# myshell-ai/OpenVoice

Measured on NVIDIA H100. Metric: audio_seconds_per_second, higher is better.
Workload: dtype f32 (3xFP16 split-precision tensor-core convs with fp32 accumulation, fp32 FFMA elsewhere)

## Files before the change

include/ovc.h:

```cpp
#ifndef OVC_B200_H
#define OVC_B200_H

#include <stddef.h>
#include <stdint.h>

#ifdef __cplusplus
extern "C" {
#endif

#define OVC_ABI_VERSION 11

#if defined(__GNUC__)
#define OVC_API __attribute__((visibility("default")))
#else
#define OVC_API
#endif

enum {
  OVC_OK = 0,
  OVC_ERR_INVALID = -1,
  OVC_ERR_CUDA = -2,
  OVC_ERR_STATE = -3,
  OVC_ERR_MISSING = -4,
  OVC_ERR_NOMEM = -5
};

typedef struct ovc_ctx ovc_ctx;

typedef struct ovc_hparams {
  int32_t spec_channels;
  int32_t inter_channels;
  int32_t hidden_channels;
  int32_t gin_channels;
// ... 91 lines not shown
                                 const ovc_item_params* items);

OVC_API int ovc_tts_encode_state(ovc_ctx* ctx, float* stats, int32_t* cum, float* g, void* stream);

OVC_API int ovc_tts_encode_state_rows(ovc_ctx* ctx, const int64_t* dst_row, int N, int Tp, float* stats, int32_t* cum,
                                      float* g, int64_t* y_lengths, void* stream);
OVC_API int ovc_tts_state_rows(ovc_ctx* ctx, const float* stats, const int32_t* cum, const float* g, const int64_t* y_lengths,
                               int B, int T, const int64_t* dst_row, int N, int Tp, float* d_stats, int32_t* d_cum,
                               float* d_g, int64_t* d_y_lengths, void* stream);

OVC_API int ovc_tts_decode_windows(ovc_ctx* ctx, const float* stats, const int32_t* cum, const float* g,
                                   const int64_t* y_lengths, int N, int T, const int64_t* row, const int64_t* frame0,
                                   const int64_t* len, int W, int Wmax, const uint64_t* seed, const int64_t* stream,
                                   const float* noise_scale, float* o, float* z_p, void* cuda_stream);

OVC_API int ovc_set_precision(ovc_ctx* ctx, int mode);

#define OVC_OPT_TTS_SIMPLE 2
#define OVC_OPT_GRAPH 3
#define OVC_OPT_PDL 5
#define OVC_OPT_BRANCHES 7
#define OVC_OPT_PAIR 8
#define OVC_OPT_PAIR_OCC 9
OVC_API int ovc_set_option(ovc_ctx* ctx, int key, int value);

OVC_API int ovc_last_launch_count(const ovc_ctx* ctx);

OVC_API int ovc_graph_replays(const ovc_ctx* ctx);

OVC_API int ovc_profile_enable(ovc_ctx* ctx, int enable);
OVC_API int ovc_profile_read(ovc_ctx* ctx, double* ms, int64_t* launches, double* flops, double* bytes);
OVC_API int ovc_profile_detail(ovc_ctx* ctx, int max, char* names, double* ms, double* flops, double* bytes,
                               int* family);

OVC_API int ovc_debug_enable(ovc_ctx* ctx, int enable);
OVC_API int ovc_debug_fetch(ovc_ctx* ctx, const char* name, float* host_out, size_t max_floats,
                    int64_t* shape4 );

#ifdef __cplusplus
}
#endif
#endif
```

openvoice_b200/_native.py:

```python
from __future__ import annotations

import ctypes as C
import os
from typing import Dict, Iterable, Optional, Tuple

_HERE = os.path.dirname(os.path.abspath(__file__))
LIB_PATH = os.path.join(_HERE, "libovc_b200.so")

ABI_VERSION = 11
EXPORTS = (
    "ovc_abi_version", "ovc_last_error", "ovc_create", "ovc_destroy", "ovc_load_tensor",
    "ovc_finalize_weights", "ovc_workspace_floats", "ovc_voice_conversion", "ovc_last_launch_count",
    "ovc_profile_enable", "ovc_profile_read", "ovc_profile_detail", "ovc_debug_enable", "ovc_debug_fetch",
    "ovc_spectrogram", "ovc_convert_waveform", "ovc_set_precision", "ovc_reference_encoder",
    "ovc_tts_info", "ovc_tts_encode", "ovc_tts_decode", "ovc_set_option", "ovc_graph_replays",
    "ovc_reference_encoder_ragged", "ovc_resample", "ovc_resample_span", "ovc_voice_conversion_items",
    "ovc_convert_waveform_items", "ovc_tts_encode_items", "ovc_tts_decode_items", "ovc_philox_normals",
    "ovc_tts_encode_state", "ovc_tts_decode_windows", "ovc_spectrogram_ring", "ovc_splice",
    "ovc_tts_encode_state_rows", "ovc_tts_state_rows",
)

STREAM_OPEN = 2 ** 63 - 1
SPLICE_PCM16 = 1


class OvcHParams(C.Structure):
    _fields_ = [
        ("spec_channels", C.c_int32), ("inter_channels", C.c_int32), ("hidden_channels", C.c_int32),
        ("gin_channels", C.c_int32), ("resblock", C.c_int32), ("n_resblock_kernels", C.c_int32),
        ("resblock_kernel_sizes", C.c_int32 * 4), ("resblock_dilations", (C.c_int32 * 3) * 4),
        ("n_upsamples", C.c_int32), ("upsample_rates", C.c_int32 * 4),
        ("upsample_kernel_sizes", C.c_int32 * 4), ("upsample_initial_channel", C.c_int32),
# ... 208 lines not shown
        used, ignored = [], []
        for k, v in sd.items():
            a = v.detach().cpu().float().contiguous().numpy() if hasattr(v, "detach") else np.ascontiguousarray(v, dtype=np.float32)
            if a.ndim == 0 or a.ndim > 4:
                ignored.append(k)
                continue
            shape = (C.c_int64 * a.ndim)(*a.shape)
            rc = self.lib.ovc_load_tensor(self.handle, k.encode(), a.ctypes.data_as(C.c_void_p), shape, a.ndim)
            _check(self.lib, rc, f"ovc_load_tensor({k})")
            (ignored if rc == 1 else used).append(k)
        self.finalized = False
        return used, ignored

    def finalize(self):
        _check(self.lib, self.lib.ovc_finalize_weights(self.handle), "ovc_finalize_weights")
        self.finalized = True

    def set_precision(self, mode: str):
        m = PRECISIONS[mode]
        _check(self.lib, self.lib.ovc_set_precision(self.handle, m), "ovc_set_precision")
        self.precision = mode

    def set_option(self, key: str, value: int):
        k = {"tts_simple": 2, "graph": 3, "pdl": 5, "branches": 7, "pair": 8, "pair_occ": 9}[key]
        _check(self.lib, self.lib.ovc_set_option(self.handle, k, int(value)), "ovc_set_option")

    def voice_conversion(self, spec, lengths, g_src, g_tgt, noise=None, tau: float = 0.3, seed: int = 0,
                         ragged: bool = False, latents: bool = True, stream=None, items: Optional[dict] = None, out=None):
        import torch
        assert spec.is_cuda and spec.dtype == torch.float32 and spec.is_contiguous()
        assert lengths.is_cuda and lengths.dtype == torch.int64 and lengths.is_contiguous()
        B, S, T = spec.shape
        gs = g_src.reshape(B, -1).contiguous().float()
        gt = g_tgt.reshape(B, -1).contiguous().float()
        if noise is not None:
            noise = noise.contiguous().float()
            assert tuple(noise.shape) == (B, self.hp.inter_channels, T)
        hop = self.hp.hop_length
        if out is not None:
            assert out.is_cuda and out.dtype == torch.float32 and out.is_contiguous() and out.numel() == B * hop * T
            o = out.view(B, 1, hop * T)
        else:
            o = torch.empty(B, 1, hop * T, device=spec.device, dtype=torch.float32)
        lat = None
        if latents:
            lat = tuple(torch.empty(B, self.hp.inter_channels, T, device=spec.device, dtype=torch.float32)
                        for _ in range(3))
# ... 332 lines not shown
```

openvoice_b200/csrc/ovc_lib.cu:

```cuda
#include <cuda_runtime.h>

#include <algorithm>
#include <cmath>
#include <cstdarg>
#include <cstdio>
#include <cstdlib>
#include <cstring>
#include <map>
#include <string>
#include <vector>

#include "../../include/ovc.h"
#include "ovc_convpack.h"
#include "ovc_small.cuh"
#include "ovc_tcconv.cuh"
#include "ovc_tts.cuh"
#include "ovc_refenc.cuh"
#include "ovc_resample.cuh"
#include "ovc_splice.h"
#include "ovc_variants.h"

namespace ovc {

static thread_local std::string g_err;
// ... 126 lines not shown
  bool finalized = false;

  float* d_w = nullptr;
  size_t w_floats = 0;
  std::vector<float> h_w;

  ConvLayer enc_pre, enc_pre16, enc_proj;
  WNLayers enc_wn;
  ConvLayer flow_pre[4], flow_post[4];
  WNLayers flow_wn[4];
  ConvLayer dec_pre, dec_ups[4];
  ConvLayer rb_c1[12][3], rb_c2[12][3];
  TcLayer tc_c1[12][3], tc_c2[12][3], tc_ups[4], tc_pre;
  float* d_tcw = nullptr;
  std::vector<float> h_tcw;
  int precision = 0;
  bool tts_simple = false;
  bool use_graph = true;
  int use_pdl = 2;
  bool use_branches = true;
  int par_frames = 512;
  bool use_pair = true;
  bool use_pair_occ = true;
  bool pair_occ2_ok[TCN_N_OCC2] = {};
  cudaStream_t br_stream[2] = {nullptr, nullptr};
  cudaEvent_t br_ev[4] = {nullptr, nullptr, nullptr, nullptr};
  size_t post_w_off = 0;
  size_t cond_w_off = 0, cond_b_off = 0;
  int* d_cond_wrow = nullptr;
  int* d_cond_sel = nullptr;
  int cond_rows_out = 0;
  int cond_off_enc = 0, cond_off_fsrc = 0, cond_off_ftgt = 0, cond_off_dec = 0;
  int cond_off_enc_tc = 0, cond_off_fsrc_tc = 0, cond_off_ftgt_tc = 0;

  float2* d_tw = nullptr;
  float* d_win = nullptr;

  bool has_refenc = false;
  size_t re_conv_w[6] = {0}, re_conv_b[6] = {0}, re_wih = 0, re_whh = 0, re_bih = 0, re_bhh = 0, re_pw = 0, re_pb = 0,
         re_lng = 0, re_lnb = 0;
  int re_gru_in = 0;
  float* d_re = nullptr;
  size_t re_floats = 0;

  std::map<std::pair<int64_t, int64_t>, double*> rs_banks;
  bool rs_smem_opt_in = false;
// ... 365 lines not shown
        {"ref_enc.gru.weight_ih_l0", {384, c->re_gru_in}, &c->re_wih}, {"ref_enc.gru.weight_hh_l0", {384, 128}, &c->re_whh},
        {"ref_enc.gru.bias_ih_l0", {384}, &c->re_bih},                 {"ref_enc.gru.bias_hh_l0", {384}, &c->re_bhh},
        {"ref_enc.proj.weight", {G, 128}, &c->re_pw},                  {"ref_enc.proj.bias", {G}, &c->re_pb},
        {"ref_enc.layernorm.weight", {S}, &c->re_lng},                 {"ref_enc.layernorm.bias", {S}, &c->re_lnb}};
    for (const auto& e : re) {
      const HostTensor* t;
      TRY(tensor(c, e.key, e.shape, &t));
      *e.off = append(c->h_w, t->data);
    }
    c->has_refenc = true;
  }
  c->tts = TtsLayers();
  if (find(c, "enc_p.emb.weight")) TRY(pack_tts(c));
  ON_DEVICE(c);
  if (c->d_w) { cudaFree(c->d_w); c->d_w = nullptr; }
  c->w_floats = c->h_w.size();
  CK(cudaMalloc(&c->d_w, c->w_floats * sizeof(float)));
  CK(cudaMemcpy(c->d_w, c->h_w.data(), c->w_floats * sizeof(float), cudaMemcpyHostToDevice));
  if (c->d_tcw) { cudaFree(c->d_tcw); c->d_tcw = nullptr; }
  CK(cudaMalloc(&c->d_tcw, c->h_tcw.size() * sizeof(float)));
  CK(cudaMemcpy(c->d_tcw, c->h_tcw.data(), c->h_tcw.size() * sizeof(float), cudaMemcpyHostToDevice));
  c->h_tcw.clear();
  c->h_tcw.shrink_to_fit();
  CK(cudaFuncSetAttribute(tcconv_kernel<128, false>, cudaFuncAttributeMaxDynamicSharedMemorySize, (int)TcnCfg<128, false>::SMEM_BYTES));
  CK(cudaFuncSetAttribute(tcconv_kernel<64, false>, cudaFuncAttributeMaxDynamicSharedMemorySize, (int)TcnCfg<64, false>::SMEM_BYTES));
  CK(cudaFuncSetAttribute(tcconv_kernel<32, false>, cudaFuncAttributeMaxDynamicSharedMemorySize, (int)TcnCfg<32, false>::SMEM_BYTES));
  CK(cudaFuncSetAttribute(tcconv_kernel<128, true>, cudaFuncAttributeMaxDynamicSharedMemorySize, (int)TcnCfg<128, true>::SMEM_BYTES));
  CK(cudaFuncSetAttribute(tcconv_kernel<64, true>, cudaFuncAttributeMaxDynamicSharedMemorySize, (int)TcnCfg<64, true>::SMEM_BYTES));
  CK(cudaFuncSetAttribute(tcconv_kernel<32, true>, cudaFuncAttributeMaxDynamicSharedMemorySize, (int)TcnCfg<32, true>::SMEM_BYTES));
  for (int i = 0; i < TCN_N_OCC2; ++i) {
    const TcPairKernel k = tc_pair_kernel(kTcPairOcc2[i].C, kTcPairOcc2[i].o);
    CK(cudaFuncSetAttribute(k.fn, cudaFuncAttributeMaxDynamicSharedMemorySize, (int)k.smem));
    int blocks = 0;
    CK(cudaOccupancyMaxActiveBlocksPerMultiprocessor(&blocks, k.fn, TCN_THREADS, k.smem));
    c->pair_occ2_ok[i] = blocks >= 2;
    if (blocks < 2)
      fprintf(stderr, "ovc: the C = %d conv-pair kernel with %d operand buffer(s) fits %d CTA(s) per SM, not 2; its pairs run "
              "one CTA per SM\n", kTcPairOcc2[i].C, kTcPairOcc2[i].o.nabuf, blocks);
  }
  if (c->d_cond_wrow) cudaFree(c->d_cond_wrow);
  if (c->d_cond_sel) cudaFree(c->d_cond_sel);
  CK(cudaMalloc(&c->d_cond_wrow, wrow.size() * sizeof(int)));
  CK(cudaMalloc(&c->d_cond_sel, sel.size() * sizeof(int)));
  CK(cudaMemcpy(c->d_cond_wrow, wrow.data(), wrow.size() * sizeof(int), cudaMemcpyHostToDevice));
  CK(cudaMemcpy(c->d_cond_sel, sel.data(), sel.size() * sizeof(int), cudaMemcpyHostToDevice));
  if (!c->d_tw) {
    std::vector<float2> tw(STFT_N);
    std::vector<float> win(STFT_N);
    const double PI = 3.14159265358979323846;
    for (int m = 0; m < STFT_N; ++m) {
      tw[m] = make_float2((float)std::cos(2.0 * PI * m / STFT_N), (float)(-std::sin(2.0 * PI * m / STFT_N)));
      win[m] = (float)(0.5 - 0.5 * std::cos(2.0 * PI * m / STFT_N));
    }
    CK(cudaMalloc(&c->d_tw, STFT_N * sizeof(float2)));
    CK(cudaMalloc(&c->d_win, STFT_N * sizeof(float)));
    CK(cudaMemcpy(c->d_tw, tw.data(), STFT_N * sizeof(float2), cudaMemcpyHostToDevice));
    CK(cudaMemcpy(c->d_win, win.data(), STFT_N * sizeof(float), cudaMemcpyHostToDevice));
// ... 175 lines not shown
static int launch_tc(Run& r, const TcLayer& T, const float* x, float* y, const float* res, int t_len, int mul, float slope,
                     float scale, int accumulate, int family, const TcExtra& ex = TcExtra()) {
  TcConvArgs a{};
  const int y_ld = ex.y_ld ? ex.y_ld : T.Ntot;
  a.x = x; a.x_bs = (long long)T.Cin * r.P * mul;
  a.w = reinterpret_cast<const uint16_t*>(r.c->d_tcw + T.w_off);
  a.bias = ex.bias ? ex.bias : r.c->d_tcw + T.b_off; a.bias_bs = ex.bias_bs;
  a.y = y; a.y_bs = (long long)y_ld * r.P * mul; a.y_ld = y_ld;
  a.r = res;
  a.s = ex.s; a.s_bs = a.y_bs;
  a.epi = ex.epi; a.split = ex.split; a.first = ex.first;
  a.lens = ex.use_lens_frames ? r.lens : r.glens; a.tmax = r.Tmax; a.mul = mul;
  a.lens_x = ex.lens_x; a.has_lens_x = ex.has_lens_x ? 1 : 0;
  a.Cin = T.Cin; a.Ntot = T.Ntot; a.K = T.K; a.DIL = T.DIL;
  a.slope = slope; a.scale = scale; a.accumulate = accumulate;
  a.passes = r.c->precision == 2 ? 1 : 3;
  if (T.TN == 0) return fail(OVC_ERR_INVALID, "conv %d -> %d (k %d, dilation %d) does not fit the tensor-core kernels", T.Cin, T.Ntot, T.K, T.DIL);
  if (!(slope >= 0.f && slope <= 1.f)) return fail(OVC_ERR_INVALID, "leaky_relu slope %g outside [0, 1]", (double)slope);
  TRY(prof_begin(r));
  const TcGrid g = tc_grid(t_len, r.B, T.Ntot, T.TN, r.c->sm_count, ex.grid_div);
  const int n_tt = g.n_tt, total = g.total;
  dim3 pg((unsigned)g.grid_x, g.ncol, 1);
  const bool pdl = r.c->use_pdl == 1 || (r.c->use_pdl == 2 && ex.epi != 0);
  if (T.TN == 128) CK(launch_ex(tcconv_kernel<128, false>, pg, TCN_THREADS, TcnCfg<128, false>::SMEM_BYTES, r.st, pdl, a, n_tt, total));
  else if (T.TN == 64) CK(launch_ex(tcconv_kernel<64, false>, pg, TCN_THREADS, TcnCfg<64, false>::SMEM_BYTES, r.st, pdl, a, n_tt, total));
  else CK(launch_ex(tcconv_kernel<32, false>, pg, TCN_THREADS, TcnCfg<32, false>::SMEM_BYTES, r.st, pdl, a, n_tt, total));
  CK(cudaGetLastError());
  r.c->launches++;
  const double units = (double)r.B * t_len;
  const int eff_k = family == 2 ? 2 : T.K;
  TRY(prof_end(r, T.TN == 128 ? V_TC128 : T.TN == 64 ? V_TC64 : V_TC32, family == 1 ? 1 : 0, 2.0 * T.Cin * T.Ntot * eff_k * units,
               4.0 * (T.Cin + T.Ntot * (1 + (res ? 1 : 0) + (accumulate ? 1 : 0))) * units, (T.Cin << 16) | (T.K << 8) | T.DIL));
  return OVC_OK;
}

static int launch_pair(Run& r, const TcLayer& T1, const TcLayer& T2, const float* x, float* y, int t_len, int mul, float slope,
                       float scale, int accumulate) {
  TcConvArgs a{};
  const int C = T1.TN;
  a.x = x; a.x_bs = (long long)C * r.P * mul;
  a.w = reinterpret_cast<const uint16_t*>(r.c->d_tcw + T1.w_off);
  a.w2 = reinterpret_cast<const uint16_t*>(r.c->d_tcw + T2.w_off);
  a.bias = r.c->d_tcw + T1.b_off; a.bias2 = r.c->d_tcw + T2.b_off;
  a.y = y; a.y_bs = a.x_bs; a.y_ld = C;
  a.lens = r.glens; a.tmax = r.Tmax; a.mul = mul;
  a.Cin = C; a.Ntot = C; a.K = T1.K; a.DIL = T1.DIL;
  a.slope = slope; a.scale = scale; a.accumulate = accumulate;
  a.passes = r.c->precision == 2 ? 1 : 3;
  TcPairOcc o = r.c->use_pair_occ ? tc_pair_occ(T1, T2) : TcPairOcc();
  for (int i = 0; i < TCN_N_OCC2; ++i)
    if (o.occ == 2 && kTcPairOcc2[i].C == C && kTcPairOcc2[i].o.nabuf == o.nabuf && !r.c->pair_occ2_ok[i]) o = TcPairOcc();
  const TcPairKernel k = tc_pair_kernel(C, o);
  if (!k.fn) return fail(OVC_ERR_INVALID, "no conv-pair kernel for C = %d at %d CTA(s) per SM, %d operand buffer(s)", C, o.occ, o.nabuf);
  const TcGrid g = tc_pair_grid(t_len, r.B, T1.K, r.c->sm_count, o.occ);
  const int n_tt = g.n_tt, total = g.total;
  TRY(prof_begin(r));
  dim3 pg((unsigned)g.grid_x, 1, 1);
  CK(launch_ex(k.fn, pg, TCN_THREADS, k.smem, r.st, false, a, n_tt, total));
  CK(cudaGetLastError());
  r.c->launches++;
  const double units = (double)r.B * t_len;
  TRY(prof_end(r, C == 128 ? V_TCPAIR128 : C == 64 ? V_TCPAIR64 : V_TCPAIR32, 1, 2.0 * 2.0 * C * C * T1.K * units, 4.0 * C * (2 + (accumulate ? 1 : 0)) * units,
               (C << 16) | (T1.K << 8) | T1.DIL));
  return OVC_OK;
}

static int launch_transpose(Run& r, const float* src, float* dst, int rows, int cols) {
  dim3 grid((cols + 31) / 32, (rows + 31) / 32, r.B);
  TRY(prof_begin(r));
  transpose_kernel<<<grid, 256, 0, r.st>>>(src, dst, rows, cols, (long long)rows * cols);
  CK(cudaGetLastError());
  r.c->launches++;
  TRY(prof_end(r, V_TRANSPOSE, 0, 0.0, 8.0 * rows * cols * r.B));
  return OVC_OK;
}

static int run_wn(Run& r, const WNLayers& wn, float* x, float* skip, float* acts, const float* cond, int cond_bs) {
  const int P = r.P, T = r.Tmax;
  const long long bs = 192LL * P;
  const int n = (int)wn.in.size();
  for (int i = 0; i < n; ++i) {
// ... 138 lines not shown
  }
  const cudaError_t ie = cudaGraphInstantiate(&e->exec, graph, 0);
  cudaGraphDestroy(graph);
  if (ie != cudaSuccess) {
    cudaGetLastError();
    e->exec = nullptr;
    e->seen = -1000000;
    return body(st);
  }
  e->launches = c->launches;
  CK(cudaGraphLaunch(e->exec, st));
  c->graph_replays++;
  return OVC_OK;
}

static int set_call_params(ovc_ctx* c, uint64_t seed, float tau, const ItemParams& items, cudaStream_t st) {
  if (!c->d_callp) CK(cudaMalloc(&c->d_callp, sizeof(CallParams)));
  set_call_params_kernel<<<1, 1, 0, st>>>(c->d_callp, seed, tau, items);
  CK(cudaGetLastError());
  return OVC_OK;
}
static uintptr_t option_bits(const ovc_ctx* c) {
  return (uintptr_t)c->precision | ((uintptr_t)c->use_pdl << 15) | ((uintptr_t)c->use_branches << 14) | ((uintptr_t)c->use_pair << 17) |
         ((uintptr_t)c->use_pair_occ << 18);
}

static int ensure_ws(ovc_ctx* c, const WsLayout& W, int B, int Tmax, cudaStream_t st) {
  if (W.total <= c->ws_floats) return OVC_OK;
  CK(cudaStreamSynchronize(st));
  drop_graphs(c);
  if (c->d_ws) CK(cudaFree(c->d_ws));
  c->d_ws = nullptr;
  c->ws_floats = 0;
  cudaError_t e = cudaMalloc(&c->d_ws, W.total * sizeof(float));
  if (e != cudaSuccess) {
    cudaGetLastError();
    return fail(OVC_ERR_NOMEM, "workspace of %.2f GB for B=%d Tmax=%d does not fit: %s", W.total * 4e-9, B, Tmax,
                cudaGetErrorString(e));
  }
  c->ws_floats = W.total;
  return OVC_OK;
}

static int copy_latent_out(Run& r, const WsLayout& W, float* ws, float* dst) {
  if (!dst) return OVC_OK;
  dim3 grid((r.Tmax + 255) / 256, 192, r.B);
  copy_latent_kernel<<<grid, 256, 0, r.st>>>(ws + W.z, W.P, dst, r.Tmax, 192, r.lens);
// ... 727 lines not shown
  CK(cudaGetLastError());
  return OVC_OK;
}

int ovc_set_precision(ovc_ctx* c, int mode) {
  if (!c) return fail(OVC_ERR_INVALID, "null context");
  if (mode < 0 || mode > 2) return fail(OVC_ERR_INVALID, "precision mode must be 0 (fp32 FFMA), 1 (3xFP16 tensor cores) or 2 (single-pass fp16)");
  c->precision = mode;
  return OVC_OK;
}

int ovc_set_option(ovc_ctx* c, int key, int value) {
  if (!c) return fail(OVC_ERR_INVALID, "null context");
  switch (key) {
    case OVC_OPT_TTS_SIMPLE: c->tts_simple = value != 0; return OVC_OK;
    case OVC_OPT_GRAPH: c->use_graph = value != 0; return OVC_OK;
    case OVC_OPT_PDL:
      if (value < 0 || value > 2) return fail(OVC_ERR_INVALID, "pdl must be 0, 1 or 2");
      c->use_pdl = value;
      return OVC_OK;
    case OVC_OPT_BRANCHES: c->use_branches = value != 0; return OVC_OK;
    case OVC_OPT_PAIR: c->use_pair = value != 0; return OVC_OK;
    case OVC_OPT_PAIR_OCC: c->use_pair_occ = value != 0; return OVC_OK;
    default: return fail(OVC_ERR_INVALID, "unknown option %d", key);
  }
}

int ovc_last_launch_count(const ovc_ctx* c) { return c ? c->launches : 0; }

int ovc_graph_replays(const ovc_ctx* c) { return c ? c->graph_replays : 0; }

int ovc_profile_enable(ovc_ctx* c, int enable) {
  if (!c) return fail(OVC_ERR_INVALID, "null context");
  c->prof = enable != 0;
  c->ev_used = 0;
  c->ev_flops.clear();
  c->ev_bytes.clear();
  c->ev_variant.clear();
  c->ev_family.clear();
  c->ev_tag.clear();
  return OVC_OK;
}

int ovc_profile_read(ovc_ctx* c, double* ms, int64_t* launches, double* flops, double* bytes) {
  if (!c) return fail(OVC_ERR_INVALID, "null context");
  double tms = 0, tf = 0, tb = 0;
// ... 68 lines not shown
```

openvoice_b200/csrc/ovc_tcconv.cuh:

```cuda
#pragma once
#include "ovc_conv.cuh"
#include "ovc_tc.cuh"
#include "ovc_tcpack.h"

namespace ovc {

struct TcConvArgs {
  const float* x; long long x_bs;
  const uint16_t* w;
  const float* bias; long long bias_bs;
  float* y; long long y_bs; int y_ld;
  const float* r;
  float* s; long long s_bs;
  int epi;
  int split; int first;
  const long long* lens; int tmax; int mul;
  const long long* lens_x; int has_lens_x;
  int Cin; int Ntot; int K; int DIL;
  float slope; float scale; int accumulate;
  int passes;
  const uint16_t* w2; const float* bias2;
};

__device__ __forceinline__ void pdl_launch_dependents() { asm volatile("griddepcontrol.launch_dependents;" ::: "memory"); }
__device__ __forceinline__ void pdl_wait() { asm volatile("griddepcontrol.wait;" ::: "memory"); }

__device__ __forceinline__ void mbar_arrive(uint64_t* bar) {
  asm volatile("mbarrier.arrive.shared::cta.b64 _, [%0];" ::"r"(smem_u32(bar)) : "memory");
}
__device__ __forceinline__ void named_bar_sync(int id, int threads) {
  asm volatile("bar.sync %0, %1;" ::"r"(id), "r"(threads) : "memory");
}

template <int TN>
__device__ __forceinline__ void tc_epilogue(const TcConvArgs& a, const float (&d)[TN], int b, int t0, int n0, int lim, int row_a) {
  const int csub = (threadIdx.x & 3) * 2;
  float* yb = a.y + (size_t)b * a.y_bs;
  const float* rb = a.r ? a.r + (size_t)b * a.y_bs : nullptr;
  float* sb = a.s ? a.s + (size_t)b * a.s_bs : nullptr;
  const float* bias = a.bias + (size_t)b * a.bias_bs;
  const bool two = a.passes == 3;
  const int ta = t0 + row_a, tb = ta + 8;
  const bool oka = ta < lim, okb = tb < lim;
#pragma unroll
  for (int c0 = 0; c0 < TN; c0 += 32) {
    float v[16];
#pragma unroll
    for (int i = 0; i < 16; ++i) v[i] = two ? fmaf(d[TN / 2 + c0 / 2 + i], tc::kLoInv, d[c0 / 2 + i]) : d[c0 / 2 + i];
#pragma unroll
    for (int g = 0; g < 4; ++g) {
      const float2 bq = __ldg(reinterpret_cast<const float2*>(bias + n0 + c0 + 8 * g + csub));
      v[4 * g] += bq.x; v[4 * g + 1] += bq.y; v[4 * g + 2] += bq.x; v[4 * g + 3] += bq.y;
    }
    if (a.epi == 0) {
      float* ypa = yb + (size_t)ta * a.y_ld + n0 + c0 + csub;
      float* ypb = yb + (size_t)tb * a.y_ld + n0 + c0 + csub;
      const float* rpa = rb ? rb + (size_t)ta * a.y_ld + n0 + c0 + csub : nullptr;
      const float* rpb = rb ? rb + (size_t)tb * a.y_ld + n0 + c0 + csub : nullptr;
#pragma unroll
      for (int g = 0; g < 4; ++g) {
        float2 oa = make_float2(v[4 * g], v[4 * g + 1]), ob = make_float2(v[4 * g + 2], v[4 * g + 3]);
        if (rb) {
          const float2 qa = oka ? *reinterpret_cast<const float2*>(rpa + 8 * g) : make_float2(0.f, 0.f);
          const float2 qb = okb ? *reinterpret_cast<const float2*>(rpb + 8 * g) : make_float2(0.f, 0.f);
          oa.x += qa.x; oa.y += qa.y; ob.x += qb.x; ob.y += qb.y;
        }
        if (a.accumulate) {
          const float2 ya = oka ? *reinterpret_cast<const float2*>(ypa + 8 * g) : make_float2(0.f, 0.f);
          const float2 yc = okb ? *reinterpret_cast<const float2*>(ypb + 8 * g) : make_float2(0.f, 0.f);
          oa.x = ya.x + oa.x; oa.y = ya.y + oa.y;
          ob.x = yc.x + ob.x; ob.y = yc.y + ob.y;
// ... 14 lines not shown
        if (oka) *reinterpret_cast<float2*>(ypa + 8 * g) = oa;
        if (okb) *reinterpret_cast<float2*>(ypb + 8 * g) = ob;
      }
    } else {
      const int col = n0 + c0;
      const bool to_x = col < a.split;
      const bool add = to_x || !a.first;
      float* dst = (to_x ? yb + col : sb + (col - a.split)) + csub;
#pragma unroll
      for (int g = 0; g < 4; ++g) {
        float2 oa = make_float2(v[4 * g], v[4 * g + 1]), ob = make_float2(v[4 * g + 2], v[4 * g + 3]);
        if (add) {
          const float2 qa = oka ? *reinterpret_cast<const float2*>(dst + (size_t)ta * a.y_ld + 8 * g) : make_float2(0.f, 0.f);
          const float2 qb = okb ? *reinterpret_cast<const float2*>(dst + (size_t)tb * a.y_ld + 8 * g) : make_float2(0.f, 0.f);
          oa = make_float2(qa.x + oa.x, qa.y + oa.y);
          ob = make_float2(qb.x + ob.x, qb.y + ob.y);
        }
        if (oka) *reinterpret_cast<float2*>(dst + (size_t)ta * a.y_ld + 8 * g) = oa;
        if (okb) *reinterpret_cast<float2*>(dst + (size_t)tb * a.y_ld + 8 * g) = ob;
      }
    }
  }
}

template <int TN>
__device__ __forceinline__ void tc_mma_step(float (&d)[TN], uint64_t a_hi, uint64_t a_lo, uint64_t b, bool three, bool first) {
  float (&lo)[TN / 2] = *reinterpret_cast<float(*)[TN / 2]>(&d[TN / 2]);
  float (&hi)[TN / 2] = *reinterpret_cast<float(*)[TN / 2]>(&d[0]);
  tc::Wgmma<TN>::mma(hi, a_hi, b, first ? 0 : 1);
  if (three) {
    tc::Wgmma<TN>::mma(lo, a_hi, b + TN, first ? 0 : 1);
    tc::Wgmma<TN>::mma(lo, a_lo, b, 1);
  }
}

constexpr int TCN_THREADS = 384;
constexpr int TCN_NCT = 96;

template <int TN, bool PAIR, int OCC = 1, int NAB = 2>
struct TcnCfg {
  static_assert(!PAIR || TN == 32 || TN == 64 || TN == 128, "conv pairs: C = 32, 64 or 128");
  static_assert(OCC == 1 || (PAIR && TN <= 64), "two CTAs per SM: C = 32 / 64 pairs");
  static constexpr int KCH = 32, NKC = KCH / 8;
  static constexpr int ROWS = 194;
  static constexpr int ROWS2 = TCN_ROWS2;
  static constexpr int NABUF = NAB;
  static constexpr int RING = PAIR ? tc_pair_ring(TN, OCC, NAB) : tc_ring_slots(TN, PAIR);
  static constexpr int SLOT_BYTES = 2 * 2 * TN * 16;
  static constexpr int A_BUF_BYTES = 2 * NKC * ROWS * 16;
  static constexpr int A2_BYTES = PAIR ? 2 * (TN / 8) * ROWS2 * 16 : 0;
  static constexpr size_t SMEM_BYTES = 1024 + NABUF * A_BUF_BYTES + A2_BYTES + RING * SLOT_BYTES;
  static_assert(!PAIR || SMEM_BYTES == tc_pair_smem(TN, NABUF, RING), "tc_pair_smem");
  static_assert(SMEM_BYTES <= (OCC == 1 ? 232448 : TCN_SMEM_OCC2), "shared memory budget");
  static_assert((2 * NABUF + 2 * RING) * 8 <= 1024, "barrier area");
  static constexpr int PROD_REGS = OCC == 1 ? 56 : 32, MMA_REGS = OCC == 1 ? 224 : 104;
};

template <int TN, bool PAIR, int OCC = 1, int NAB = 2>
__global__ void __launch_bounds__(TCN_THREADS, OCC) tcconv_kernel(const TcConvArgs a, int n_tt, int total) {
  using Cfg = TcnCfg<TN, PAIR, OCC, NAB>;
  constexpr int ROWS = Cfg::ROWS, ROWS2 = Cfg::ROWS2, NABUF = Cfg::NABUF, RING = Cfg::RING, NKC = Cfg::NKC;
  extern __shared__ __align__(128) unsigned char smem_raw[];
  uint64_t* bars = reinterpret_cast<uint64_t*>(smem_raw);
  uint64_t *a_full = bars, *a_empty = bars + NABUF, *b_full = a_empty + NABUF, *b_empty = b_full + RING;
  unsigned char* abuf = smem_raw + 1024;
  unsigned char* a2buf = abuf + NABUF * Cfg::A_BUF_BYTES;
  unsigned char* bring = a2buf + Cfg::A2_BYTES;

  const int tid = threadIdx.x, lane = tid & 31;
  const int warp = __shfl_sync(0xffffffffu, tid >> 5, 0);
  const int H1 = (a.K - 1) / 2 * a.DIL;
  const int H2 = PAIR ? (a.K - 1) / 2 : 0;
  const int R = 128 - 2 * H2;
  const int rows8 = (128 + 2 * H1 + 7) & ~7;
  const int nq = a.Cin / Cfg::KCH;
  const int n_slots = (a.Cin / 16) * a.K;
  const int n_w = PAIR ? 2 * n_slots : n_slots;
  const bool resident = n_w <= RING;
  if (H1 > TCN_HMAX || (PAIR && 128 + 2 * H2 > ROWS2)) __trap();
  constexpr uint32_t BYTES = Cfg::SLOT_BYTES;

  if (tid == 0) {
    for (int i = 0; i < NABUF; ++i) { mbar_init(&a_full[i], TCN_NCT); mbar_init(&a_empty[i], 2); }
    for (int i = 0; i < RING; ++i) { mbar_init(&b_full[i], 1); mbar_init(&b_empty[i], 2); }
    fence_mbar_init();
  }
  if (PAIR) {
    for (int i = tid; i < Cfg::A2_BYTES / 16; i += TCN_THREADS) reinterpret_cast<uint4*>(a2buf)[i] = make_uint4(0u, 0u, 0u, 0u);
    asm volatile("fence.proxy.async.shared::cta;" ::: "memory");
  }
  __syncthreads();
  pdl_launch_dependents();
  if (warp != 0) pdl_wait();

#define TCN_FOR_TILES                                                                                   \
  for (int tile = blockIdx.x; tile < total; tile += gridDim.x) {                                        \
    const int b = tile / n_tt, t0 = (tile % n_tt) * R;                                                  \
    const int lim = (a.lens ? (int)min((long long)a.tmax, a.lens[b]) : a.tmax) * a.mul;                 \
    const int lim_x = a.has_lens_x ? (int)min((long long)a.tmax, a.lens_x[b]) * a.mul : lim;            \
    (void)lim_x;                                                                                        \
    if (t0 >= lim) continue;

  if (warp < 4) {
    tc::regs_dealloc<Cfg::PROD_REGS>();
    if (warp == 0) {
      if (lane == 0) {
        const unsigned char* wt = reinterpret_cast<const unsigned char*>(a.w) + (size_t)blockIdx.y * n_slots * BYTES;
        if (resident) {
          for (int it = 0; it < n_w; ++it) {
            const unsigned char* src = it < n_slots ? wt + (size_t)it * BYTES
                                                    : reinterpret_cast<const unsigned char*>(a.w2) + (size_t)(it - n_slots) * BYTES;
// ... 42 lines not shown
              if (i < items && t >= 0 && t < lim_x) {
                const float4* src = reinterpret_cast<const float4*>(xb + (size_t)t * a.Cin + q * Cfg::KCH + kc * 8);
                v0[u] = src[0];
                v1[u] = src[1];
              }
            }
#pragma unroll
            for (int u = 0; u < PB; ++u) {
              const int i = i0 + TCN_NCT * u;
              if (i >= items) break;
              const int row = i >> 2, kc = i & 3;
              uint4 hi, lo;
              tc::split_f16x8(v0[u], v1[u], a.slope, hi, lo);
              *reinterpret_cast<uint4*>(ah + (kc * ROWS + row) * 16) = hi;
              *reinterpret_cast<uint4*>(al + (kc * ROWS + row) * 16) = lo;
            }
          }
          asm volatile("fence.proxy.async.shared::cta;" ::: "memory");
          mbar_arrive(&a_full[buf]);
          if (++buf == NABUF) { buf = 0; ephase ^= 1; }
        }
      }
    }
  } else {
    tc::regs_alloc<Cfg::MMA_REGS>();
    const int wg = (warp >> 2) - 1;
    const bool leader = (tid & 127) == 0;
    const int row_a = 64 * wg + 16 * (warp & 3) + (lane >> 2);
    constexpr uint32_t LBO_A = ROWS * 16, LBO_A2 = ROWS2 * 16, LBO_B = 2 * TN * 16, SBO = 128;
    constexpr uint32_t A_LO16 = (NKC * ROWS * 16) >> 4, A2_LO16 = ((TN / 8) * ROWS2 * 16) >> 4, SLOT16 = BYTES >> 4;
    const uint64_t a_proto = tc::make_desc(0, LBO_A, SBO), b_proto = tc::make_desc(0, LBO_B, SBO);
    const uint64_t b_ring = b_proto + (tc::smem_addr(bring) >> 4);
    const bool three = a.passes == 3;
    float d[TN];
#pragma unroll
    for (int i = 0; i < TN; ++i) d[i] = 0.f;
    if (resident)
      for (int it = 0; it < n_w; ++it) mbar_wait(&b_full[it], 0u);
    int slot = 0, buf = 0;
    uint32_t bphase = 0, aphase = 0;
    TCN_FOR_TILES
      (void)lim_x;
      bool first = true;
      if (resident) slot = 0;
      for (int q = 0; q < nq; ++q) {
        mbar_wait(&a_full[buf], aphase);
        tc::fence_regs(d);
        tc::wgmma_fence();
        int prev = -1;
        for (int j = 0; j < 2; ++j) {
          uint64_t a_cur = a_proto + ((tc::smem_addr(abuf + buf * Cfg::A_BUF_BYTES) + 64 * wg * 16 + 2 * j * LBO_A) >> 4);
          for (int tap = 0; tap < a.K; ++tap) {
            if (!resident) mbar_wait(&b_full[slot], bphase);
            tc_mma_step<TN>(d, a_cur, a_cur + A_LO16, b_ring + (uint32_t)slot * SLOT16, three, first);
            tc::wgmma_commit();
            if (!resident) {
              tc::wgmma_wait<1>();
              if (leader && prev >= 0) mbar_arrive(&b_empty[prev]);
              prev = slot;
            }
            first = false;
            a_cur += a.DIL;
            if (++slot == RING) { slot = 0; bphase ^= 1; }
          }
        }
        tc::wgmma_wait<0>();
        tc::fence_regs(d);
        if (leader) {
          if (prev >= 0) mbar_arrive(&b_empty[prev]);
          mbar_arrive(&a_empty[buf]);
        }
        if (++buf == NABUF) { buf = 0; aphase ^= 1; }
      }
      if constexpr (!PAIR) {
        tc_epilogue<TN>(a, d, b, t0, blockIdx.y * TN, lim, row_a);
      } else {
        named_bar_sync(1, 256);
        unsigned char* a2h = a2buf;
        unsigned char* a2l = a2buf + (TN / 8) * ROWS2 * 16;
        const int ta = t0 - H2 + row_a, tb = ta + 8;
        const bool oka = ta >= 0 && ta < lim, okb = tb >= 0 && tb < lim;
        const int csub = (lane & 3) * 2;
#pragma unroll
        for (int g = 0; g < TN / 8; ++g) {
          const float2 bq = __ldg(reinterpret_cast<const float2*>(a.bias + 8 * g + csub));
          float x[4];
#pragma unroll
          for (int i = 0; i < 4; ++i) x[i] = (three ? fmaf(d[TN / 2 + 4 * g + i], tc::kLoInv, d[4 * g + i]) : d[4 * g + i]) + ((i & 1) ? bq.y : bq.x);
          x[0] = oka ? fmaxf(x[0], x[0] * a.slope) : 0.f;
          x[1] = oka ? fmaxf(x[1], x[1] * a.slope) : 0.f;
          x[2] = okb ? fmaxf(x[2], x[2] * a.slope) : 0.f;
          x[3] = okb ? fmaxf(x[3], x[3] * a.slope) : 0.f;
          const __half2 ha = __floats2half2_rn(x[0], x[1]), hb = __floats2half2_rn(x[2], x[3]);
          const float2 fa = __half22float2(ha), fb = __half22float2(hb);
          const __half2 la = __floats2half2_rn((x[0] - fa.x) * tc::kLoScale, (x[1] - fa.y) * tc::kLoScale);
          const __half2 lb = __floats2half2_rn((x[2] - fb.x) * tc::kLoScale, (x[3] - fb.y) * tc::kLoScale);
          const int oa = (g * ROWS2 + row_a) * 16 + (lane & 3) * 4, ob = oa + 8 * 16;
          *reinterpret_cast<__half2*>(a2h + oa) = ha;
          *reinterpret_cast<__half2*>(a2h + ob) = hb;
          *reinterpret_cast<__half2*>(a2l + oa) = la;
// ... 8 lines not shown
        int prev = -1;
        for (int kk = 0; kk < TN / 16; ++kk) {
          uint64_t a_cur = a2_proto + ((tc::smem_addr(a2buf) + 64 * wg * 16 + 2 * kk * LBO_A2) >> 4);
          for (int tap = 0; tap < a.K; ++tap) {
            if (resident) {
              tc_mma_step<TN>(d, a_cur, a_cur + A2_LO16, b_ring + (uint32_t)(n_slots + kk * a.K + tap) * SLOT16, three, first2);
            } else {
              mbar_wait(&b_full[slot], bphase);
              tc_mma_step<TN>(d, a_cur, a_cur + A2_LO16, b_ring + (uint32_t)slot * SLOT16, three, first2);
              tc::wgmma_commit();
              tc::wgmma_wait<1>();
              if (leader && prev >= 0) mbar_arrive(&b_empty[prev]);
              prev = slot;
              if (++slot == RING) { slot = 0; bphase ^= 1; }
            }
            first2 = false;
            a_cur += 1;
          }
        }
        tc::wgmma_commit();
        tc::wgmma_wait<0>();
        tc::fence_regs(d);
        if (leader && prev >= 0) mbar_arrive(&b_empty[prev]);
        TcConvArgs e = a;
        e.y_ld = TN; e.r = a.x; e.bias = a.bias2; e.bias_bs = 0; e.epi = 0;
        tc_epilogue<TN>(e, d, b, t0, 0, min(lim, t0 + R), row_a);
      }
    }
  }
#undef TCN_FOR_TILES
}

struct TcPairKernel {
  void (*fn)(TcConvArgs, int, int) = nullptr;
  size_t smem = 0;
};
inline TcPairKernel tc_pair_kernel(int C, TcPairOcc o) {
  if (o.occ == 1 && o.nabuf == 2) {
    if (C == 128) return {tcconv_kernel<128, true>, TcnCfg<128, true>::SMEM_BYTES};
    if (C == 64) return {tcconv_kernel<64, true>, TcnCfg<64, true>::SMEM_BYTES};
    if (C == 32) return {tcconv_kernel<32, true>, TcnCfg<32, true>::SMEM_BYTES};
  } else if (o.occ == 2) {
    if (C == 32 && o.nabuf == 2) return {tcconv_kernel<32, true, 2, 2>, TcnCfg<32, true, 2, 2>::SMEM_BYTES};
    if (C == 32 && o.nabuf == 1) return {tcconv_kernel<32, true, 2, 1>, TcnCfg<32, true, 2, 1>::SMEM_BYTES};
    if (C == 64 && o.nabuf == 1) return {tcconv_kernel<64, true, 2, 1>, TcnCfg<64, true, 2, 1>::SMEM_BYTES};
  }
  return {};
}
constexpr int TCN_N_OCC2 = 3;
constexpr struct { int C; TcPairOcc o; } kTcPairOcc2[TCN_N_OCC2] = {{32, {2, 2}}, {32, {2, 1}}, {64, {2, 1}}};

template <int C>
__global__ void __launch_bounds__(256) conv_post_cl_kernel(const float* __restrict__ x, long long x_bs,
                                                           const float* __restrict__ w, float* __restrict__ y,
                                                           long long y_bs, int y_len, const long long* lens, int tmax,
                                                           int mul) {
  constexpr int TB = 256, ROWS = TB + 6, LD = ROWS + 3;
  __shared__ float ws[7][C];
  __shared__ float xs[C][LD];
  for (int i = threadIdx.x; i < C * 7; i += blockDim.x) ws[i % 7][i / 7] = w[i];
  const int b = blockIdx.y;
  const int lim = (lens ? (int)min((long long)tmax, lens[b]) : tmax) * mul;
  const int t0 = blockIdx.x * TB;
  const float* xb = x + (size_t)b * x_bs;
  for (int idx = threadIdx.x; idx < ROWS * (C / 4); idx += blockDim.x) {
    const int row = idx / (C / 4), q = idx % (C / 4);
    const int tt = t0 - 3 + row;
    float4 v = make_float4(0.f, 0.f, 0.f, 0.f);
// ... 40 lines not shown
```

Baseline: 2312.

## Add warp-specialized staged epilogue for TN=128 tensor-core convs

Adds a fourth warpgroup of store warps to the TN=128 conv and conv-pair kernels. The MMA warps now write their finished accumulators to a shared-memory staging tile and signal an mbarrier, and the store warps run the bias, activation and residual epilogue while the MMA warps start the next tile. The aim is to overlap epilogue global stores with tensor-core work. In exchange, MMA registers drop from 224 to 184, producer registers shrink, more shared memory is used, and extra barrier syncs are added. It is enabled by default only when passes*K >= 15.

```diff
diff --git a/include/ovc.h b/include/ovc.h
--- a/include/ovc.h
+++ b/include/ovc.h
@@ -8,7 +8,7 @@
 extern "C" {
 #endif
 
-#define OVC_ABI_VERSION 11
+#define OVC_ABI_VERSION 12
 
 #if defined(__GNUC__)
 #define OVC_API __attribute__((visibility("default")))
@@ -146,6 +146,7 @@
 #define OVC_OPT_BRANCHES 7
 #define OVC_OPT_PAIR 8
 #define OVC_OPT_PAIR_OCC 9
+#define OVC_OPT_STAGED_EPI 10
 OVC_API int ovc_set_option(ovc_ctx* ctx, int key, int value);
 
 OVC_API int ovc_last_launch_count(const ovc_ctx* ctx);
diff --git a/openvoice_b200/_native.py b/openvoice_b200/_native.py
--- a/openvoice_b200/_native.py
+++ b/openvoice_b200/_native.py
@@ -7,7 +7,7 @@
 _HERE = os.path.dirname(os.path.abspath(__file__))
 LIB_PATH = os.path.join(_HERE, "libovc_b200.so")
 
-ABI_VERSION = 11
+ABI_VERSION = 12
 EXPORTS = (
     "ovc_abi_version", "ovc_last_error", "ovc_create", "ovc_destroy", "ovc_load_tensor",
     "ovc_finalize_weights", "ovc_workspace_floats", "ovc_voice_conversion", "ovc_last_launch_count",
@@ -262,7 +262,7 @@
         self.precision = mode
 
     def set_option(self, key: str, value: int):
-        k = {"tts_simple": 2, "graph": 3, "pdl": 5, "branches": 7, "pair": 8, "pair_occ": 9}[key]
+        k = {"tts_simple": 2, "graph": 3, "pdl": 5, "branches": 7, "pair": 8, "pair_occ": 9, "staged_epi": 10}[key]
         _check(self.lib, self.lib.ovc_set_option(self.handle, k, int(value)), "ovc_set_option")
 
     def voice_conversion(self, spec, lengths, g_src, g_tgt, noise=None, tau: float = 0.3, seed: int = 0,
diff --git a/openvoice_b200/csrc/ovc_lib.cu b/openvoice_b200/csrc/ovc_lib.cu
--- a/openvoice_b200/csrc/ovc_lib.cu
+++ b/openvoice_b200/csrc/ovc_lib.cu
@@ -172,6 +172,7 @@
   int par_frames = 512;
   bool use_pair = true;
   bool use_pair_occ = true;
+  bool use_staged_epi = true;
   bool pair_occ2_ok[TCN_N_OCC2] = {};
   cudaStream_t br_stream[2] = {nullptr, nullptr};
   cudaEvent_t br_ev[4] = {nullptr, nullptr, nullptr, nullptr};
@@ -583,17 +584,17 @@
   CK(cudaMemcpy(c->d_tcw, c->h_tcw.data(), c->h_tcw.size() * sizeof(float), cudaMemcpyHostToDevice));
   c->h_tcw.clear();
   c->h_tcw.shrink_to_fit();
-  CK(cudaFuncSetAttribute(tcconv_kernel<128, false>, cudaFuncAttributeMaxDynamicSharedMemorySize, (int)TcnCfg<128, false>::SMEM_BYTES));
-  CK(cudaFuncSetAttribute(tcconv_kernel<64, false>, cudaFuncAttributeMaxDynamicSharedMemorySize, (int)TcnCfg<64, false>::SMEM_BYTES));
-  CK(cudaFuncSetAttribute(tcconv_kernel<32, false>, cudaFuncAttributeMaxDynamicSharedMemorySize, (int)TcnCfg<32, false>::SMEM_BYTES));
-  CK(cudaFuncSetAttribute(tcconv_kernel<128, true>, cudaFuncAttributeMaxDynamicSharedMemorySize, (int)TcnCfg<128, true>::SMEM_BYTES));
-  CK(cudaFuncSetAttribute(tcconv_kernel<64, true>, cudaFuncAttributeMaxDynamicSharedMemorySize, (int)TcnCfg<64, true>::SMEM_BYTES));
-  CK(cudaFuncSetAttribute(tcconv_kernel<32, true>, cudaFuncAttributeMaxDynamicSharedMemorySize, (int)TcnCfg<32, true>::SMEM_BYTES));
+  for (int TN : {128, 64, 32})
+    for (bool staged : {false, true}) {
+      const TcKernel k = tc_conv_kernel(TN, staged), p = tc_pair_kernel(TN, TcPairOcc(), staged);
+      CK(cudaFuncSetAttribute(k.fn, cudaFuncAttributeMaxDynamicSharedMemorySize, (int)k.smem));
+      CK(cudaFuncSetAttribute(p.fn, cudaFuncAttributeMaxDynamicSharedMemorySize, (int)p.smem));
+    }
   for (int i = 0; i < TCN_N_OCC2; ++i) {
-    const TcPairKernel k = tc_pair_kernel(kTcPairOcc2[i].C, kTcPairOcc2[i].o);
+    const TcKernel k = tc_pair_kernel(kTcPairOcc2[i].C, kTcPairOcc2[i].o);
     CK(cudaFuncSetAttribute(k.fn, cudaFuncAttributeMaxDynamicSharedMemorySize, (int)k.smem));
     int blocks = 0;
-    CK(cudaOccupancyMaxActiveBlocksPerMultiprocessor(&blocks, k.fn, TCN_THREADS, k.smem));
+    CK(cudaOccupancyMaxActiveBlocksPerMultiprocessor(&blocks, k.fn, k.threads, k.smem));
     c->pair_occ2_ok[i] = blocks >= 2;
     if (blocks < 2)
       fprintf(stderr, "ovc: the C = %d conv-pair kernel with %d operand buffer(s) fits %d CTA(s) per SM, not 2; its pairs run "
@@ -815,9 +816,8 @@
   const int n_tt = g.n_tt, total = g.total;
   dim3 pg((unsigned)g.grid_x, g.ncol, 1);
   const bool pdl = r.c->use_pdl == 1 || (r.c->use_pdl == 2 && ex.epi != 0);
-  if (T.TN == 128) CK(launch_ex(tcconv_kernel<128, false>, pg, TCN_THREADS, TcnCfg<128, false>::SMEM_BYTES, r.st, pdl, a, n_tt, total));
-  else if (T.TN == 64) CK(launch_ex(tcconv_kernel<64, false>, pg, TCN_THREADS, TcnCfg<64, false>::SMEM_BYTES, r.st, pdl, a, n_tt, total));
-  else CK(launch_ex(tcconv_kernel<32, false>, pg, TCN_THREADS, TcnCfg<32, false>::SMEM_BYTES, r.st, pdl, a, n_tt, total));
+  const TcKernel k = tc_conv_kernel(T.TN, r.c->use_staged_epi && tc_stage_pays(T.K, a.passes));
+  CK(launch_ex(k.fn, pg, k.threads, k.smem, r.st, pdl, a, n_tt, total));
   CK(cudaGetLastError());
   r.c->launches++;
   const double units = (double)r.B * t_len;
@@ -843,13 +843,13 @@
   TcPairOcc o = r.c->use_pair_occ ? tc_pair_occ(T1, T2) : TcPairOcc();
   for (int i = 0; i < TCN_N_OCC2; ++i)
     if (o.occ == 2 && kTcPairOcc2[i].C == C && kTcPairOcc2[i].o.nabuf == o.nabuf && !r.c->pair_occ2_ok[i]) o = TcPairOcc();
-  const TcPairKernel k = tc_pair_kernel(C, o);
+  const TcKernel k = tc_pair_kernel(C, o, r.c->use_staged_epi && tc_stage_pays(T1.K, a.passes));
   if (!k.fn) return fail(OVC_ERR_INVALID, "no conv-pair kernel for C = %d at %d CTA(s) per SM, %d operand buffer(s)", C, o.occ, o.nabuf);
   const TcGrid g = tc_pair_grid(t_len, r.B, T1.K, r.c->sm_count, o.occ);
   const int n_tt = g.n_tt, total = g.total;
   TRY(prof_begin(r));
   dim3 pg((unsigned)g.grid_x, 1, 1);
-  CK(launch_ex(k.fn, pg, TCN_THREADS, k.smem, r.st, false, a, n_tt, total));
+  CK(launch_ex(k.fn, pg, k.threads, k.smem, r.st, false, a, n_tt, total));
   CK(cudaGetLastError());
   r.c->launches++;
   const double units = (double)r.B * t_len;
@@ -1034,7 +1034,7 @@
 }
 static uintptr_t option_bits(const ovc_ctx* c) {
   return (uintptr_t)c->precision | ((uintptr_t)c->use_pdl << 15) | ((uintptr_t)c->use_branches << 14) | ((uintptr_t)c->use_pair << 17) |
-         ((uintptr_t)c->use_pair_occ << 18);
+         ((uintptr_t)c->use_pair_occ << 18) | ((uintptr_t)c->use_staged_epi << 19);
 }
 
 static int ensure_ws(ovc_ctx* c, const WsLayout& W, int B, int Tmax, cudaStream_t st) {
@@ -1808,6 +1808,7 @@
     case OVC_OPT_BRANCHES: c->use_branches = value != 0; return OVC_OK;
     case OVC_OPT_PAIR: c->use_pair = value != 0; return OVC_OK;
     case OVC_OPT_PAIR_OCC: c->use_pair_occ = value != 0; return OVC_OK;
+    case OVC_OPT_STAGED_EPI: c->use_staged_epi = value != 0; return OVC_OK;
     default: return fail(OVC_ERR_INVALID, "unknown option %d", key);
   }
 }
diff --git a/openvoice_b200/csrc/ovc_tcconv.cuh b/openvoice_b200/csrc/ovc_tcconv.cuh
--- a/openvoice_b200/csrc/ovc_tcconv.cuh
+++ b/openvoice_b200/csrc/ovc_tcconv.cuh
@@ -31,22 +31,29 @@
 __device__ __forceinline__ void named_bar_sync(int id, int threads) {
   asm volatile("bar.sync %0, %1;" ::"r"(id), "r"(threads) : "memory");
 }
+__device__ __forceinline__ void named_bar_arrive(int id, int threads) {
+  asm volatile("bar.arrive %0, %1;" ::"r"(id), "r"(threads) : "memory");
+}
 
 template <int TN>
-__device__ __forceinline__ void tc_epilogue(const TcConvArgs& a, const float (&d)[TN], int b, int t0, int n0, int lim, int row_a) {
+__device__ __forceinline__ float tc_result(const float (&d)[TN], bool two, int j) {
+  return two ? fmaf(d[TN / 2 + j], tc::kLoInv, d[j]) : d[j];
+}
+
+template <int TN, class V>
+__device__ __forceinline__ void tc_epilogue_v(const TcConvArgs& a, V v_at, int b, int t0, int n0, int lim, int row_a) {
   const int csub = (threadIdx.x & 3) * 2;
   float* yb = a.y + (size_t)b * a.y_bs;
   const float* rb = a.r ? a.r + (size_t)b * a.y_bs : nullptr;
   float* sb = a.s ? a.s + (size_t)b * a.s_bs : nullptr;
   const float* bias = a.bias + (size_t)b * a.bias_bs;
-  const bool two = a.passes == 3;
   const int ta = t0 + row_a, tb = ta + 8;
   const bool oka = ta < lim, okb = tb < lim;
 #pragma unroll
   for (int c0 = 0; c0 < TN; c0 += 32) {
     float v[16];
 #pragma unroll
-    for (int i = 0; i < 16; ++i) v[i] = two ? fmaf(d[TN / 2 + c0 / 2 + i], tc::kLoInv, d[c0 / 2 + i]) : d[c0 / 2 + i];
+    for (int i = 0; i < 16; ++i) v[i] = v_at(c0 / 2 + i);
 #pragma unroll
     for (int g = 0; g < 4; ++g) {
       const float2 bq = __ldg(reinterpret_cast<const float2*>(bias + n0 + c0 + 8 * g + csub));
@@ -107,6 +114,16 @@
     }
   }
 }
+template <int TN>
+__device__ __forceinline__ void tc_epilogue(const TcConvArgs& a, const float (&d)[TN], int b, int t0, int n0, int lim, int row_a) {
+  const bool two = a.passes == 3;
+  tc_epilogue_v<TN>(a, [&](int j) { return tc_result<TN>(d, two, j); }, b, t0, n0, lim, row_a);
+}
+__device__ __forceinline__ TcConvArgs tc_pair_epilogue_args(const TcConvArgs& a, int TN) {
+  TcConvArgs e = a;
+  e.y_ld = TN; e.r = a.x; e.bias = a.bias2; e.bias_bs = 0; e.epi = 0;
+  return e;
+}
 
 template <int TN>
 __device__ __forceinline__ void tc_mma_step(float (&d)[TN], uint64_t a_hi, uint64_t a_lo, uint64_t b, bool three, bool first) {
@@ -122,10 +139,12 @@
 constexpr int TCN_THREADS = 384;
 constexpr int TCN_NCT = 96;
 
-template <int TN, bool PAIR, int OCC = 1, int NAB = 2>
+template <int TN, bool PAIR, int OCC = 1, int NAB = 2, bool STAGED = false>
 struct TcnCfg {
   static_assert(!PAIR || TN == 32 || TN == 64 || TN == 128, "conv pairs: C = 32, 64 or 128");
   static_assert(OCC == 1 || (PAIR && TN <= 64), "two CTAs per SM: C = 32 / 64 pairs");
+  static_assert(!STAGED || (TN == 128 && OCC == 1), "staged epilogue: TN = 128, one CTA per SM");
+  static constexpr int THREADS = STAGED ? TCN_THREADS + 128 : TCN_THREADS;
   static constexpr int KCH = 32, NKC = KCH / 8;
   static constexpr int ROWS = 194;
   static constexpr int ROWS2 = TCN_ROWS2;
@@ -134,23 +153,30 @@
   static constexpr int SLOT_BYTES = 2 * 2 * TN * 16;
   static constexpr int A_BUF_BYTES = 2 * NKC * ROWS * 16;
   static constexpr int A2_BYTES = PAIR ? 2 * (TN / 8) * ROWS2 * 16 : 0;
-  static constexpr size_t SMEM_BYTES = 1024 + NABUF * A_BUF_BYTES + A2_BYTES + RING * SLOT_BYTES;
+  static constexpr int STAGE_BYTES = STAGED ? (TN / 2) * 256 * 4 : 0;
+  static_assert(!STAGED || !PAIR || STAGE_BYTES <= A2_BYTES, "a pair's staging tile lies in its conv-2 operand");
+  static constexpr int SBUF_BYTES = STAGED && !PAIR ? STAGE_BYTES : 0;
+  static constexpr size_t SMEM_BYTES = 1024 + NABUF * A_BUF_BYTES + A2_BYTES + RING * SLOT_BYTES + SBUF_BYTES;
   static_assert(!PAIR || SMEM_BYTES == tc_pair_smem(TN, NABUF, RING), "tc_pair_smem");
   static_assert(SMEM_BYTES <= (OCC == 1 ? 232448 : TCN_SMEM_OCC2), "shared memory budget");
-  static_assert((2 * NABUF + 2 * RING) * 8 <= 1024, "barrier area");
-  static constexpr int PROD_REGS = OCC == 1 ? 56 : 32, MMA_REGS = OCC == 1 ? 224 : 104;
+  static_assert((2 * NABUF + 2 * RING + 2) * 8 <= 1024, "barrier area");
+  static constexpr int PROD_REGS = OCC == 1 && !STAGED ? 56 : 32, MMA_REGS = STAGED ? 184 : OCC == 1 ? 224 : 104;
+  static constexpr int STORE_REGS = 112;
+  static_assert(128 * PROD_REGS + 256 * MMA_REGS + (STAGED ? 128 * STORE_REGS : 0) <= 65536 / OCC, "register budget");
 };
 
-template <int TN, bool PAIR, int OCC = 1, int NAB = 2>
-__global__ void __launch_bounds__(TCN_THREADS, OCC) tcconv_kernel(const TcConvArgs a, int n_tt, int total) {
-  using Cfg = TcnCfg<TN, PAIR, OCC, NAB>;
+template <int TN, bool PAIR, int OCC = 1, int NAB = 2, bool STAGED = false>
+__global__ void __launch_bounds__(TcnCfg<TN, PAIR, OCC, NAB, STAGED>::THREADS, OCC) tcconv_kernel(const TcConvArgs a, int n_tt, int total) {
+  using Cfg = TcnCfg<TN, PAIR, OCC, NAB, STAGED>;
   constexpr int ROWS = Cfg::ROWS, ROWS2 = Cfg::ROWS2, NABUF = Cfg::NABUF, RING = Cfg::RING, NKC = Cfg::NKC;
   extern __shared__ __align__(128) unsigned char smem_raw[];
   uint64_t* bars = reinterpret_cast<uint64_t*>(smem_raw);
   uint64_t *a_full = bars, *a_empty = bars + NABUF, *b_full = a_empty + NABUF, *b_empty = b_full + RING;
+  uint64_t *s_full = b_empty + RING, *s_empty = s_full + 1;
   unsigned char* abuf = smem_raw + 1024;
   unsigned char* a2buf = abuf + NABUF * Cfg::A_BUF_BYTES;
   unsigned char* bring = a2buf + Cfg::A2_BYTES;
+  float* stage = reinterpret_cast<float*>(PAIR ? a2buf : bring + RING * Cfg::SLOT_BYTES);
 
   const int tid = threadIdx.x, lane = tid & 31;
   const int warp = __shfl_sync(0xffffffffu, tid >> 5, 0);
@@ -168,10 +194,11 @@
   if (tid == 0) {
     for (int i = 0; i < NABUF; ++i) { mbar_init(&a_full[i], TCN_NCT); mbar_init(&a_empty[i], 2); }
     for (int i = 0; i < RING; ++i) { mbar_init(&b_full[i], 1); mbar_init(&b_empty[i], 2); }
+    if (STAGED) { mbar_init(s_full, 256); mbar_init(s_empty, 128); }
     fence_mbar_init();
   }
   if (PAIR) {
-    for (int i = tid; i < Cfg::A2_BYTES / 16; i += TCN_THREADS) reinterpret_cast<uint4*>(a2buf)[i] = make_uint4(0u, 0u, 0u, 0u);
+    for (int i = tid; i < Cfg::A2_BYTES / 16; i += Cfg::THREADS) reinterpret_cast<uint4*>(a2buf)[i] = make_uint4(0u, 0u, 0u, 0u);
     asm volatile("fence.proxy.async.shared::cta;" ::: "memory");
   }
   __syncthreads();
@@ -260,6 +287,24 @@
         }
       }
     }
+  } else if (STAGED && warp >= 12) {
+    tc::regs_dealloc<Cfg::STORE_REGS>();
+    const int st = tid & 127;
+    uint32_t phase = 0;
+    TCN_FOR_TILES
+      if (PAIR) named_bar_arrive(1, 384);
+      mbar_wait(s_full, phase);
+      phase ^= 1;
+#pragma unroll 1
+      for (int h = 0; h < 2; ++h) {
+        const float* sv = stage + h * 128 + st;
+        const auto v_at = [&](int j) { return sv[j * 256]; };
+        const int row_a = 64 * h + 16 * (warp & 3) + (lane >> 2);
+        if constexpr (PAIR) tc_epilogue_v<TN>(tc_pair_epilogue_args(a, TN), v_at, b, t0, 0, min(lim, t0 + R), row_a);
+        else tc_epilogue_v<TN>(a, v_at, b, t0, blockIdx.y * TN, lim, row_a);
+      }
+      if (!PAIR) mbar_arrive(s_empty);
+    }
   } else {
     tc::regs_alloc<Cfg::MMA_REGS>();
     const int wg = (warp >> 2) - 1;
@@ -273,6 +318,13 @@
     float d[TN];
 #pragma unroll
     for (int i = 0; i < TN; ++i) d[i] = 0.f;
+    const auto stage_tile = [&]() {
+#pragma unroll
+      for (int j = 0; j < TN / 2; ++j) stage[j * 256 + tid - 128] = tc_result<TN>(d, three, j);
+      mbar_arrive(s_full);
+    };
+    uint32_t sphase = 1;
+    (void)sphase;
     if (resident)
       for (int it = 0; it < n_w; ++it) mbar_wait(&b_full[it], 0u);
     int slot = 0, buf = 0;
@@ -311,9 +363,15 @@
         if (++buf == NABUF) { buf = 0; aphase ^= 1; }
       }
       if constexpr (!PAIR) {
-        tc_epilogue<TN>(a, d, b, t0, blockIdx.y * TN, lim, row_a);
+        if constexpr (STAGED) {
+          mbar_wait(s_empty, sphase);
+          sphase ^= 1;
+          stage_tile();
+        } else {
+          tc_epilogue<TN>(a, d, b, t0, blockIdx.y * TN, lim, row_a);
+        }
       } else {
-        named_bar_sync(1, 256);
+        named_bar_sync(1, STAGED ? 384 : 256);
         unsigned char* a2h = a2buf;
         unsigned char* a2l = a2buf + (TN / 8) * ROWS2 * 16;
         const int ta = t0 - H2 + row_a, tb = ta + 8;
@@ -368,28 +426,45 @@
         tc::wgmma_wait<0>();
         tc::fence_regs(d);
         if (leader && prev >= 0) mbar_arrive(&b_empty[prev]);
-        TcConvArgs e = a;
-        e.y_ld = TN; e.r = a.x; e.bias = a.bias2; e.bias_bs = 0; e.epi = 0;
-        tc_epilogue<TN>(e, d, b, t0, 0, min(lim, t0 + R), row_a);
+        if constexpr (STAGED) {
+          named_bar_sync(3, 256);
+          stage_tile();
+        } else {
+          tc_epilogue<TN>(tc_pair_epilogue_args(a, TN), d, b, t0, 0, min(lim, t0 + R), row_a);
+        }
       }
     }
   }
 #undef TCN_FOR_TILES
 }
 
-struct TcPairKernel {
+struct TcKernel {
   void (*fn)(TcConvArgs, int, int) = nullptr;
   size_t smem = 0;
+  int threads = 0;
 };
-inline TcPairKernel tc_pair_kernel(int C, TcPairOcc o) {
+using TcPairKernel = TcKernel;
+template <int TN, bool PAIR, int OCC = 1, int NAB = 2, bool STAGED = false>
+inline TcKernel tc_kernel() {
+  using Cfg = TcnCfg<TN, PAIR, OCC, NAB, STAGED>;
+  return {tcconv_kernel<TN, PAIR, OCC, NAB, STAGED>, Cfg::SMEM_BYTES, Cfg::THREADS};
+}
+inline bool tc_stage_pays(int K, int passes) { return passes * K >= 15; }
+inline TcKernel tc_conv_kernel(int TN, bool staged) {
+  if (TN == 128) return staged ? tc_kernel<128, false, 1, 2, true>() : tc_kernel<128, false>();
+  if (TN == 64) return tc_kernel<64, false>();
+  if (TN == 32) return tc_kernel<32, false>();
+  return {};
+}
+inline TcKernel tc_pair_kernel(int C, TcPairOcc o, bool staged = false) {
   if (o.occ == 1 && o.nabuf == 2) {
-    if (C == 128) return {tcconv_kernel<128, true>, TcnCfg<128, true>::SMEM_BYTES};
-    if (C == 64) return {tcconv_kernel<64, true>, TcnCfg<64, true>::SMEM_BYTES};
-    if (C == 32) return {tcconv_kernel<32, true>, TcnCfg<32, true>::SMEM_BYTES};
+    if (C == 128) return staged ? tc_kernel<128, true, 1, 2, true>() : tc_kernel<128, true>();
+    if (C == 64) return tc_kernel<64, true>();
+    if (C == 32) return tc_kernel<32, true>();
   } else if (o.occ == 2) {
-    if (C == 32 && o.nabuf == 2) return {tcconv_kernel<32, true, 2, 2>, TcnCfg<32, true, 2, 2>::SMEM_BYTES};
-    if (C == 32 && o.nabuf == 1) return {tcconv_kernel<32, true, 2, 1>, TcnCfg<32, true, 2, 1>::SMEM_BYTES};
-    if (C == 64 && o.nabuf == 1) return {tcconv_kernel<64, true, 2, 1>, TcnCfg<64, true, 2, 1>::SMEM_BYTES};
+    if (C == 32 && o.nabuf == 2) return tc_kernel<32, true, 2, 2>();
+    if (C == 32 && o.nabuf == 1) return tc_kernel<32, true, 2, 1>();
+    if (C == 64 && o.nabuf == 1) return tc_kernel<64, true, 2, 1>();
   }
   return {};
 }
```

Result: faster. 2391 (median of 6 runs) (+3.4%).
